# LLNL/ppo_and_friends

Hardware: AMD Instinct MI355X
Metric: env_steps_per_sec (higher is better)
Workload: dtype f32; 1 GPU; C2 CartPole-v1 MLP (4->128x3->2 actor, ->1 critic), envs_per_proc=4096, ts_per_rollout=128, fixed-length synthetic trajectories, batch_size=256, epochs_per_iter=10; parallelism=dp1, hip_graphs=True

## Files before the change

ppo_and_friends_amd/csrc/mlp_device.hpp:

```cpp
#pragma once
#include <type_traits>
#include "common.hpp"
#include <cfloat>

namespace ppoaf {

constexpr int kRows = PPOAF_UPDATE_ROWS_PER_WG;
constexpr int kMaxLayers = 8;
constexpr int kMaxOut = 16;
constexpr int kMaxAdvLds = 4096;
constexpr int kThreads = 256;

typedef float f32x4 __attribute__((ext_vector_type(4)));

struct NetDev {
    int in_dim, H, depth, out_dim, act;
    long offset, size, log_std_off;
    long offW[kMaxLayers], offB[kMaxLayers];
};

__device__ __forceinline__ float act_fwd(float z, int act) {
    if (act == PPOAF_ACT_RELU) return fmaxf(z, 0.f);
    if (act == PPOAF_ACT_LEAKY_RELU) return z > 0.f ? z : 0.01f * z;
    return tanhf(z);
// ... 63 lines not shown
#pragma unroll
    for (int c = 1; c < HT; c += 2) fr[c] = frag_u4(__builtin_amdgcn_raw_buffer_load_b128(rs, off + 64u * c, 0, 0));
}
template <int HT>
__device__ __forceinline__ void load_dgrad_frags_buf(const float* __restrict__ W, int n0, int lane, float4 (&fr)[HT]) {
    constexpr int H = 16 * HT;
    const __amdgpu_buffer_rsrc_t rs = frag_rsrc(W);
    const unsigned off = (unsigned)((4 * (lane >> 4) * H + n0 + (lane & 15)) * 4);
#pragma unroll
    for (int c = 0; c < HT; ++c) {
        const int row = 16 * c * H * 4;
        fr[c] = make_float4(__uint_as_float(__builtin_amdgcn_raw_buffer_load_b32(rs, off, row, 0)),
                            __uint_as_float(__builtin_amdgcn_raw_buffer_load_b32(rs, off, row + H * 4, 0)),
                            __uint_as_float(__builtin_amdgcn_raw_buffer_load_b32(rs, off, row + 2 * H * 4, 0)),
                            __uint_as_float(__builtin_amdgcn_raw_buffer_load_b32(rs, off, row + 3 * H * 4, 0)));
    }
}

template <int HT>
__device__ __forceinline__ f32x4 mfma_rows_x_frags(const float* __restrict__ A, int HS, int lane,
                                                   const float4 (&fr)[HT], float init) {
    const float* arow = A + (lane & 15) * HS + 4 * (lane >> 4);
    f32x4 acc0 = {init, init, init, init};
    f32x4 acc1 = {0.f, 0.f, 0.f, 0.f};
#pragma unroll
    for (int c = 0; c < HT; ++c) {
        const float4 a4 = *reinterpret_cast<const float4*>(arow + 16 * c);
        if (c & 1) {
            acc1 = __builtin_amdgcn_mfma_f32_16x16x4f32(a4.x, fr[c].x, acc1, 0, 0, 0);
            acc1 = __builtin_amdgcn_mfma_f32_16x16x4f32(a4.y, fr[c].y, acc1, 0, 0, 0);
            acc1 = __builtin_amdgcn_mfma_f32_16x16x4f32(a4.z, fr[c].z, acc1, 0, 0, 0);
            acc1 = __builtin_amdgcn_mfma_f32_16x16x4f32(a4.w, fr[c].w, acc1, 0, 0, 0);
        } else {
            acc0 = __builtin_amdgcn_mfma_f32_16x16x4f32(a4.x, fr[c].x, acc0, 0, 0, 0);
            acc0 = __builtin_amdgcn_mfma_f32_16x16x4f32(a4.y, fr[c].y, acc0, 0, 0, 0);
            acc0 = __builtin_amdgcn_mfma_f32_16x16x4f32(a4.z, fr[c].z, acc0, 0, 0, 0);
            acc0 = __builtin_amdgcn_mfma_f32_16x16x4f32(a4.w, fr[c].w, acc0, 0, 0, 0);
        }
    }
    return acc0 + acc1;
}

constexpr int kLineRow = 36;
constexpr int kLineSlot = 16 * kLineRow;
template <int HT>
__device__ __forceinline__ void load_fwd_lines_buf(const float* __restrict__ W, int n0, int lane, float4 (&raw)[HT]) {
    static_assert(HT % 2 == 0, "whole lines: H a multiple of 32");
    const __amdgpu_buffer_rsrc_t rs = frag_rsrc(W);
    const unsigned off = (unsigned)(((n0 + (lane >> 3)) * (16 * HT) + 4 * (lane & 7)) * 4);
#pragma unroll
    for (int q = 0; q < HT / 2; ++q) {
        raw[2 * q] = frag_u4(__builtin_amdgcn_raw_buffer_load_b128(rs, off + 128u * q, 0, 0));
        raw[2 * q + 1] = frag_u4(__builtin_amdgcn_raw_buffer_load_b128(rs, off + (unsigned)(8 * 16 * HT * 4) + 128u * q, 0, 0));
    }
}
template <int HT>
__device__ __forceinline__ f32x4 mfma_rows_x_lines(const float* __restrict__ A, int HS, int lane, const float4 (&raw)[HT],
                                                   float init, float* __restrict__ scratch) {
    constexpr int NL = HT / 2;
    const float* arow = A + (lane & 15) * HS + 4 * (lane >> 4);
    float* wr = scratch + (lane >> 3) * kLineRow + 4 * (lane & 7);
    const float* rd = scratch + (lane & 15) * kLineRow + 4 * (lane >> 4);
    f32x4 acc0 = {init, init, init, init};
    f32x4 acc1 = {0.f, 0.f, 0.f, 0.f};
    *reinterpret_cast<float4*>(wr) = raw[0];
    *reinterpret_cast<float4*>(wr + 8 * kLineRow) = raw[1];
    if (NL > 1) {
        *reinterpret_cast<float4*>(wr + kLineSlot) = raw[2];
        *reinterpret_cast<float4*>(wr + kLineSlot + 8 * kLineRow) = raw[3];
    }
    __builtin_amdgcn_wave_barrier();
    float4 f0 = *reinterpret_cast<const float4*>(rd);
    float4 f1 = *reinterpret_cast<const float4*>(rd + 16);
#pragma unroll
    for (int q = 0; q < NL; ++q) {
        const int slot = (q & 1) * kLineSlot;
        float4 g0 = f0, g1 = f1;
        if (q + 1 < NL) {
            g0 = *reinterpret_cast<const float4*>(rd + (kLineSlot - slot));
            g1 = *reinterpret_cast<const float4*>(rd + (kLineSlot - slot) + 16);
        }
        const float4 a0 = *reinterpret_cast<const float4*>(arow + 32 * q);
        const float4 a1 = *reinterpret_cast<const float4*>(arow + 32 * q + 16);
        acc0 = __builtin_amdgcn_mfma_f32_16x16x4f32(a0.x, f0.x, acc0, 0, 0, 0);
        acc0 = __builtin_amdgcn_mfma_f32_16x16x4f32(a0.y, f0.y, acc0, 0, 0, 0);
        acc0 = __builtin_amdgcn_mfma_f32_16x16x4f32(a0.z, f0.z, acc0, 0, 0, 0);
        acc0 = __builtin_amdgcn_mfma_f32_16x16x4f32(a0.w, f0.w, acc0, 0, 0, 0);
        acc1 = __builtin_amdgcn_mfma_f32_16x16x4f32(a1.x, f1.x, acc1, 0, 0, 0);
        acc1 = __builtin_amdgcn_mfma_f32_16x16x4f32(a1.y, f1.y, acc1, 0, 0, 0);
        acc1 = __builtin_amdgcn_mfma_f32_16x16x4f32(a1.z, f1.z, acc1, 0, 0, 0);
        acc1 = __builtin_amdgcn_mfma_f32_16x16x4f32(a1.w, f1.w, acc1, 0, 0, 0);
        __builtin_amdgcn_wave_barrier();
        if (q + 2 < NL) {
            *reinterpret_cast<float4*>(wr + slot) = raw[2 * q + 4];
            *reinterpret_cast<float4*>(wr + slot + 8 * kLineRow) = raw[2 * q + 5];
        }
        f0 = g0; f1 = g1;
    }
    return acc0 + acc1;
}

__device__ __forceinline__ void wgrad_mtile(const float* __restrict__ D, int HS, const float* __restrict__ Bsrc,
                                            int strideB, int m0, int ntiles, int n_valid, int lane,
                                            float* __restrict__ dstW, int ldw) {
    float a[4];
#pragma unroll
    for (int j = 0; j < 4; ++j) a[j] = D[(4 * (lane >> 4) + j) * HS + m0 + (lane & 15)];
    const float* bcol = Bsrc + (4 * (lane >> 4)) * strideB + (lane & 15);
    float* drow = dstW + (long)(m0 + 4 * (lane >> 4)) * ldw + (lane & 15);
#pragma unroll 4
    for (int nt = 0; nt < ntiles; ++nt) {
        f32x4 acc = {0.f, 0.f, 0.f, 0.f};
#pragma unroll
        for (int j = 0; j < 4; ++j)
            acc = __builtin_amdgcn_mfma_f32_16x16x4f32(a[j], bcol[j * strideB + 16 * nt], acc, 0, 0, 0);
        if (16 * nt + (lane & 15) < n_valid) {
#pragma unroll
            for (int r = 0; r < 4; ++r) drow[(long)r * ldw + 16 * nt] = acc[r];
        }
    }
}

template <int NT>
__device__ __forceinline__ void wgrad_mtile_full(const float* __restrict__ D, int HS, const float* __restrict__ Bsrc,
                                                 int strideB, int m0, int lane, float* __restrict__ dstW, int ldw) {
    float a[4];
#pragma unroll
    for (int j = 0; j < 4; ++j) a[j] = D[(4 * (lane >> 4) + j) * HS + m0 + (lane & 15)];
    const float* bcol = Bsrc + (4 * (lane >> 4)) * strideB + (lane & 15);
    float b[NT][4];
#pragma unroll
    for (int nt = 0; nt < NT; ++nt)
#pragma unroll
        for (int j = 0; j < 4; ++j) b[nt][j] = bcol[j * strideB + 16 * nt];
    f32x4 acc[NT];
#pragma unroll
    for (int nt = 0; nt < NT; ++nt) acc[nt] = f32x4{0.f, 0.f, 0.f, 0.f};
#pragma unroll
    for (int j = 0; j < 4; ++j)
#pragma unroll
        for (int nt = 0; nt < NT; ++nt) acc[nt] = __builtin_amdgcn_mfma_f32_16x16x4f32(a[j], b[nt][j], acc[nt], 0, 0, 0);
    float* drow = dstW + (long)(m0 + 4 * (lane >> 4)) * ldw + (lane & 15);
#pragma unroll
    for (int nt = 0; nt < NT; ++nt)
#pragma unroll
        for (int r = 0; r < 4; ++r) drow[(long)r * ldw + 16 * nt] = acc[nt][r];
}

constexpr int kNW = 8;
constexpr int kThreadsU = 64 * kNW;

template <int HT, bool ALIGNED>
__device__ __forceinline__ void load_fwd_frags_ld(const float* __restrict__ W, long ldw, int n0, int lane,
                                                  float4 (&fr)[HT]) {
    const float* w = W + (long)(n0 + (lane & 15)) * ldw + 4 * (lane >> 4);
    if (ALIGNED) {
#pragma unroll
        for (int c = 0; c < HT; c += 2) fr[c] = *reinterpret_cast<const float4*>(w + 16 * c);
        __builtin_amdgcn_sched_barrier(0);
#pragma unroll
        for (int c = 1; c < HT; c += 2) fr[c] = *reinterpret_cast<const float4*>(w + 16 * c);
    } else {
#pragma unroll
        for (int c = 0; c < HT; ++c) fr[c] = make_float4(w[16 * c], w[16 * c + 1], w[16 * c + 2], w[16 * c + 3]);
    }
}
// ... 218 lines not shown
```

ppo_and_friends_amd/csrc/ppo_update.hip:

```cpp
#include "ppo_update_fwd_bwd.hpp"
#include "peer_exchange_device.hpp"
#include <cstdlib>

namespace ppoaf {

constexpr int kRedThreads = 256;

__device__ __forceinline__ void ppo_update_bookkeeping(const UpdateDev& u);

__global__ __launch_bounds__(kRedThreads) void ppo_update_reduce_kernel(UpdateDev u, int compute_norms) {
    __shared__ double red[17];
    if (blockIdx.x == gridDim.x - 1) { ppo_update_bookkeeping(u); return; }
    const long n4 = u.bucket_total >> 2;
    const long idx = (long)blockIdx.x * kRedThreads + threadIdx.x;
    const float4* sl = reinterpret_cast<const float4*>(u.slabs);
    float4 acc = make_float4(0.f, 0.f, 0.f, 0.f);
    if (idx < n4) {
        for (int g0 = 0; g0 < u.n_wg; g0 += 8) {
            float4 v[8];
#pragma unroll
            for (int k = 0; k < 8; ++k)
                v[k] = (g0 + k < u.n_wg) ? sl[(long)(g0 + k) * n4 + idx] : make_float4(0.f, 0.f, 0.f, 0.f);
#pragma unroll
            for (int k = 0; k < 8; ++k) { acc.x += v[k].x; acc.y += v[k].y; acc.z += v[k].z; acc.w += v[k].w; }
// ... 338 lines not shown
                       dim3(kRedThreads), 0, (hipStream_t)stream, u, compute_norms);
    return check_launch("ppo_update_reduce");
}

extern "C" int ppoaf_ppo_update_reduce_exchange(const ppoaf_ppo_update_args_t* args, ppoaf_peer_exchange_t* xchg,
                                                double wait_seconds, ppoaf_stream_t stream) {
    UpdateDev u;
    int rc = make_update_dev(args, u);
    if (rc) return rc;
    PPOAF_REQUIRE(xchg && xchg->connected, "ppo_update_reduce_exchange: exchange missing or not connected");
    const long n4 = u.bucket_total >> 2;
    PPOAF_REQUIRE(xchg->dev.n4 == n4, "ppo_update_reduce_exchange: exchange made for %ld float4, bucket has %ld",
                  xchg->dev.n4, n4);
    PPOAF_REQUIRE(xchg->dev.n_ranks == u.n_ranks || !u.normalize_values, "ppo_update_reduce_exchange: %d ranks in the exchange, %d in args",
                  xchg->dev.n_ranks, u.n_ranks);
    const long groups = (n4 + kRedThreads - 1) / kRedThreads;
    PPOAF_REQUIRE(groups <= kXchgMaxGrid, "ppo_update_reduce_exchange: bucket of %ld floats needs %ld workgroups (at most %d: "
                  "use ppoaf_ppo_update_reduce + ppoaf_peer_exchange_allreduce)", (long)u.bucket_total, groups, kXchgMaxGrid);
    PPOAF_REQUIRE(wait_seconds > 0.0 && wait_seconds <= 600.0, "ppo_update_reduce_exchange: wait_seconds=%g", wait_seconds);
    hipLaunchKernelGGL(ppo_update_reduce_exchange_kernel, dim3((unsigned)groups + 1u), dim3(kRedThreads), 0,
                       (hipStream_t)stream, u, xchg->dev, (long long)(wait_seconds * 1.0e8));
    return check_launch("ppo_update_reduce_exchange");
}

extern "C" int ppoaf_ppo_update_adam(const ppoaf_ppo_update_args_t* args, int compute_norms,
                                     ppoaf_stream_t stream) {
    UpdateDev u;
    int rc = make_update_dev(args, u);
    if (rc) return rc;
    const long n4 = u.bucket_total >> 2;
    const unsigned grid = (unsigned)((n4 + 255) / 256);
    PPOAF_REQUIRE(compute_norms >= 0 && compute_norms <= 3, "ppo_update_adam: compute_norms=%d (0 .. 3)", compute_norms);
    PPOAF_REQUIRE(compute_norms != 3 || u.split, "ppo_update_adam: compute_norms = 3 follows ppoaf_ppo_update_wgrad (split_workspace set)");
    static_assert(kRedThreads == 256, "the reduce launch and the norm pass leave one partial pair per 256 float4 columns");
    if (compute_norms == 1) {
        hipLaunchKernelGGL(ppo_update_sqnorm_kernel, dim3(grid), dim3(256), 0, (hipStream_t)stream, u);
        rc = check_launch("ppo_update_adam/sqnorm");
        if (rc) return rc;
    }
    hipLaunchKernelGGL(ppo_update_adam_kernel, dim3(grid), dim3(256), 0, (hipStream_t)stream, u,
                       compute_norms == 2 ? (const double*)nullptr : (const double*)(u.norm_scratch + 6),
                       compute_norms == 3 ? (unsigned)split_wgrad_blocks(u) : grid);
    return check_launch("ppo_update_adam");
}

extern "C" int ppoaf_ppo_update_chain_allreduce(const ppoaf_ppo_update_args_t* args, ppoaf_comm_t* comm, int64_t n_minibatches,
                                                ppoaf_stream_t stream) {
    PPOAF_REQUIRE(args && comm, "ppo_update_chain_allreduce: null argument");
    PPOAF_REQUIRE(n_minibatches >= 1 && n_minibatches <= (1 << 20), "ppo_update_chain_allreduce: n_minibatches=%ld", (long)n_minibatches);
    PPOAF_REQUIRE(args->mb_offset == 0, "ppo_update_chain_allreduce: mb_offset must be 0");
    ppoaf_ppo_update_args_t a = copy_update_args(args);
    for (int64_t j = 0; j < n_minibatches; ++j) {
        a.mb_offset = j;
        a.cursor_advance = (j == n_minibatches - 1) ? n_minibatches : 0;
        int rc = ppoaf_ppo_update_fwd_bwd(&a, stream);
        if (rc == PPOAF_OK) rc = ppoaf_ppo_update_reduce(&a, 0, stream);
        if (rc == PPOAF_OK) rc = ppoaf_allreduce_sum_f32(comm, a.grads, a.bucket_total, stream);
        if (rc == PPOAF_OK) rc = ppoaf_ppo_update_adam(&a, 1, stream);
        if (rc != PPOAF_OK) return rc;
    }
    return PPOAF_OK;
}

extern "C" int ppoaf_ppo_update_adam_exchanged(const ppoaf_ppo_update_args_t* args, ppoaf_peer_exchange_t* xchg,
                                               ppoaf_stream_t stream) {
    UpdateDev u;
    int rc = make_update_dev(args, u);
    if (rc) return rc;
    PPOAF_REQUIRE(xchg && xchg->connected, "ppo_update_adam_exchanged: exchange missing or not connected");
    const long n4 = u.bucket_total >> 2;
    PPOAF_REQUIRE(xchg->dev.n4 == n4, "ppo_update_adam_exchanged: exchange made for %ld float4, bucket has %ld",
                  xchg->dev.n4, n4);
    const unsigned groups = u.split ? (unsigned)split_wgrad_blocks(u) : (unsigned)((n4 + kRedThreads - 1) / kRedThreads);
    PPOAF_REQUIRE(groups <= (unsigned)kXchgMaxGrid, "ppo_update_adam_exchanged: bucket too large for the fused exchange");
    hipLaunchKernelGGL(ppo_update_adam_kernel, dim3((unsigned)((n4 + 255) / 256)), dim3(256), 0, (hipStream_t)stream, u,
                       (const double*)xchg->dev.norm_partials, groups);
    return check_launch("ppo_update_adam_exchanged");
}

#ifdef PPOAF_STAMPS
extern "C" int ppoaf_debug_read_stamps(unsigned long long* out ) {
    return hipMemcpyFromSymbol(out, HIP_SYMBOL(g_ppo_update_stamps), sizeof(unsigned long long) * 32) == hipSuccess ? 0 : -2;
}
#endif

extern "C" int ppoaf_minibatch_moments(const float* data, const int64_t* perm, const int32_t* row_map,
                                       int64_t n_perm, int64_t B, double* records,
                                       ppoaf_stream_t stream) {
    PPOAF_REQUIRE(data && perm && records, "minibatch_moments: null pointer");
    PPOAF_REQUIRE(n_perm >= 1 && B >= 1, "minibatch_moments: n_perm=%ld B=%ld", (long)n_perm, (long)B);
    const long nb = (n_perm + B - 1) / B;
    PPOAF_REQUIRE(nb <= 0x7fffffffL, "minibatch_moments: too many mini-batches");
    hipLaunchKernelGGL(minibatch_moments_kernel, dim3((unsigned)nb), dim3(256), 0, (hipStream_t)stream,
                       data, perm, row_map, (long)n_perm, (long)B, records);
    return check_launch("minibatch_moments");
}
```

ppo_and_friends_amd/csrc/ppo_update_dev.hpp:

```cpp
#pragma once
#include "action_heads.hpp"
#include "running_stats_device.hpp"
#include "wgrad_tile.hpp"
#include <cstddef>
#include <cstring>

namespace ppoaf {

#ifdef PPOAF_STAMPS
#ifndef PPOAF_STAMP_BLOCK
#define PPOAF_STAMP_BLOCK 0
#endif
static __device__ unsigned long long g_ppo_update_stamps[2][16];
#define PPOAF_STAMP_AT(row, k, t0)                                                       \
    do {                                                                                 \
        if (blockIdx.x == PPOAF_STAMP_BLOCK && threadIdx.x == (t0)) {                    \
            unsigned long long t_;                                                       \
            asm volatile("s_memtime %0\n\ts_waitcnt lgkmcnt(0)" : "=s"(t_)::"memory");    \
            g_ppo_update_stamps[row][k] = t_;                                            \
        }                                                                                \
    } while (0)
#define PPOAF_STAMP(k) PPOAF_STAMP_AT(0, k, 0)
#define PPOAF_STAMP_W(k, w) PPOAF_STAMP_AT(1, k, 64 * (w))
#else
#define PPOAF_STAMP(k) do {} while (0)
#define PPOAF_STAMP_W(k, w) do {} while (0)
#endif

#define PPOAF_WIDTH_PAIRS_IN_UPDATE(X) X(32, 32) X(64, 64) X(128, 128) X(256, 256) X(128, 256) X(64, 128)
#define PPOAF_WIDTH_PAIRS_IN_NARROW(X) X(64, 256) X(32, 256) X(32, 64)
#define PPOAF_WIDTH_PAIRS_WIDE(X) X(256, 512)
#define PPOAF_WIDTH_PAIRS_EVERY_FORM(X) PPOAF_WIDTH_PAIRS_IN_UPDATE(X) PPOAF_WIDTH_PAIRS_IN_NARROW(X)
#define PPOAF_WIDTH_PAIRS(X) PPOAF_WIDTH_PAIRS_EVERY_FORM(X) PPOAF_WIDTH_PAIRS_WIDE(X)
#define PPOAF_WIDTH_PAIR_RUNG_(A, C) if (ppoaf_ha_ == A && ppoaf_hc_ == C) return PPOAF_WIDTH_PAIR_CALL_(A, C);
#define PPOAF_WIDTH_PAIR_LADDER_OF(LIST, ha, hc) \
    { const int ppoaf_ha_ = (ha), ppoaf_hc_ = (hc); LIST(PPOAF_WIDTH_PAIR_RUNG_) }
#define PPOAF_WIDTH_PAIR_LADDER(ha, hc) PPOAF_WIDTH_PAIR_LADDER_OF(PPOAF_WIDTH_PAIRS_EVERY_FORM, ha, hc)
#define PPOAF_WIDTH_PAIR_LADDER_ALL(ha, hc) PPOAF_WIDTH_PAIR_LADDER_OF(PPOAF_WIDTH_PAIRS, ha, hc)
inline bool width_pair_instantiated(const int ha, const int hc) {
#define PPOAF_WIDTH_PAIR_CALL_(A, C) true
    PPOAF_WIDTH_PAIR_LADDER_ALL(ha, hc)
#undef PPOAF_WIDTH_PAIR_CALL_
    return false;
}
inline bool width_pair_is_wide(const int ha, const int hc) {
#define PPOAF_WIDTH_PAIR_CALL_(A, C) true
    PPOAF_WIDTH_PAIR_LADDER_OF(PPOAF_WIDTH_PAIRS_WIDE, ha, hc)
#undef PPOAF_WIDTH_PAIR_CALL_
    return false;
}
inline size_t rowtile_wide_lds_floats(const NetDev& n) {
    const size_t HS = n.H + 4, INP = 16 * ((n.in_dim + 15) / 16) + 4;
    return 208 + (size_t)(n.depth + 1) * n.H + (size_t)n.H + kRows * INP + 3 * kRows * HS + 2 * kRows * kMaxOut;
}

struct WsDev {
    float* hbuf[2];
    float* dbuf[2];
    float* outpart[2];
    float* xbuf[2];
    int W;
    int xld[2];
    int Bp;
};

struct UpdateDev {
    NetDev net[2];
    const float* params; float* grads; float* exp_avg; float* exp_avg_sq; float* slabs;
    long bucket_total;
    int64_t* step_counts; const float* lr; double* norm_scratch;
    float beta1, beta2, adam_eps, grad_scale, max_norm; int head_kind;
    const float* obs; const float* critic_obs; const void* raw_actions;
    const float* adv; const float* old_lp; const float* rtg; float* values;
    const int64_t* perm; const int32_t* row_map; long n_rows;
    int64_t* cursor; long B, batch_stride, mb_offset, cursor_advance;
    int normalize_values, n_ranks;
    float* vn_mean; float* vn_var; double* vn_count; const double* vn_records;
    const double* adv_records;
    int normalize_adv, use_huber, pregathered;
    float surr_clip, entropy_weight, kl_loss_weight, huber_delta, min_std;
    float* loss_partials; double* totals;
    int n_wg;
    int confine;
    int split;
    WsDev sp;
    int n_slices; int slices[8];
};

inline long ws_seg_off(const NetDev& n) {
    const long szW0 = ((long)n.H * n.in_dim + 3) & ~3L;
    return n.depth == 0 ? 0 : szW0 + n.H + (long)(n.depth - 1) * ((long)n.H * n.H + n.H);
}
inline long ws_seg_len(const NetDev& n) { return n.size - ws_seg_off(n); }

inline int split_wgrad_jobs(const NetDev& n) {
    const int t = n.H / 16, t2 = (t + 1) / 2, p0 = ((n.in_dim + 15) / 16 + 1) / 2;
    return (n.depth - 1) * t * t2 + t * p0 + 1;
}
inline int split_wgrad_per_xcd(const UpdateDev& u) { return (split_wgrad_jobs(u.net[0]) + split_wgrad_jobs(u.net[1]) + 7) / 8; }
inline int split_wgrad_blocks(const UpdateDev& u) { return 8 * split_wgrad_per_xcd(u); }

inline bool args_row_pairs(const ppoaf_ppo_update_args_t* a) { return (a->row_pairs & PPOAF_SPLIT_ROW_PAIRS) != 0; }
inline bool args_wide_inputs(const ppoaf_ppo_update_args_t* a) { return (a->row_pairs & PPOAF_SPLIT_WIDE_INPUTS) != 0; }

inline int split_xld(const NetDev& n) { return n.in_dim <= 64 ? 64 : 128; }

inline size_t ws_layout(const UpdateDev& u, WsDev* ws, char* base) {
    const long Bp = (u.B + 63) & ~63L;
    size_t off = 0;
// ... 382 lines not shown
```

ppo_and_friends_amd/csrc/ppo_update_rowtile.hpp:

```cpp
#pragma once
#include "ppo_update_dev.hpp"

namespace ppoaf {

extern __shared__ __attribute__((aligned(16))) unsigned char ppo_update_smem[];




__device__ __forceinline__ int rowtile_request_args(const UpdateDev& u, int b) {
    const NetDev& a = u.net[0];
    const NetDev& c = u.net[1];
    asm("" : "+s"(b)
        : "s"(a.in_dim), "s"(a.H), "s"(a.depth), "s"(a.out_dim), "s"(a.act), "s"((&a.act)[1]), "s"(a.offset), "s"(a.size), "s"(a.log_std_off),
          "s"(c.in_dim), "s"(c.H), "s"(c.depth), "s"(c.out_dim), "s"(c.act), "s"((&c.act)[1]), "s"(c.offset), "s"(c.size), "s"(c.log_std_off),
          "s"(u.params), "s"(u.norm_scratch), "s"(u.head_kind),
          "s"(u.obs), "s"(u.critic_obs), "s"(u.raw_actions), "s"(u.adv), "s"(u.old_lp), "s"(u.rtg), "s"(u.values), "s"(u.perm),
          "s"(u.row_map), "s"(u.n_rows), "s"(u.cursor), "s"(u.B), "s"(u.batch_stride), "s"(u.mb_offset), "s"(u.cursor_advance),
          "s"(u.normalize_values), "s"(u.n_ranks), "s"(u.vn_mean), "s"(u.vn_var), "s"(u.vn_count), "s"(u.vn_records),
          "s"(u.adv_records), "s"(u.normalize_adv), "s"(u.use_huber), "s"(u.pregathered), "s"(u.surr_clip),
          "s"(u.n_wg), "s"(u.confine));
    const long cur = u.cursor[0];
    asm("" : "+s"(b)
        : "s"(cur), "s"(u.entropy_weight), "s"(u.kl_loss_weight), "s"(u.huber_delta), "s"(u.min_std), "s"(u.loss_partials),
          "s"(u.sp.hbuf[0]), "s"(u.sp.hbuf[1]), "s"(u.sp.dbuf[0]), "s"(u.sp.dbuf[1]), "s"(u.sp.outpart[0]), "s"(u.sp.outpart[1]),
          "s"(u.sp.xbuf[0]), "s"(u.sp.xbuf[1]), "s"(u.sp.W), "s"(u.sp.xld[0]), "s"(u.sp.xld[1]), "s"(u.sp.Bp), "s"(u.n_slices),
          "s"(u.slices[0]), "s"(u.slices[1]), "s"(u.slices[2]), "s"(u.slices[3]), "s"(u.slices[4]), "s"(u.slices[5]),
          "s"(u.slices[6]), "s"(u.slices[7]));
    return b;
}

template <int CP> __device__ __forceinline__ void lds_read_adjacent(const float* p, float (&v)[CP]) {
    if constexpr (CP % 4 == 0) {
#pragma unroll
        for (int q = 0; q < CP / 4; ++q) {
            const float4 t = *reinterpret_cast<const float4*>(p + 4 * q);
            v[4 * q] = t.x; v[4 * q + 1] = t.y; v[4 * q + 2] = t.z; v[4 * q + 3] = t.w;
        }
    } else {
#pragma unroll
        for (int q = 0; q < CP; ++q) v[q] = p[q];
    }
}
template <int CP> __device__ __forceinline__ void lds_write_adjacent(float* p, const float (&v)[CP]) {
    if constexpr (CP % 4 == 0) {
#pragma unroll
        for (int q = 0; q < CP / 4; ++q) *reinterpret_cast<float4*>(p + 4 * q) = make_float4(v[4 * q], v[4 * q + 1], v[4 * q + 2], v[4 * q + 3]);
    } else {
#pragma unroll
        for (int q = 0; q < CP; ++q) p[q] = v[q];
    }
}

template <int HT, bool SPLIT, bool TABLES, bool XLD = false>
__device__ __forceinline__ void ppo_update_fwd_bwd_body_as(const UpdateDev& u, const int which, const int g) {
    constexpr int H = 16 * HT, HS = H + 4;
    const int tid = threadIdx.x, lane = tid & 63, wave = tid >> 6;
    const auto& nd = u.net[which];
    const int in_dim = nd.in_dim, depth = nd.depth, out_dim = nd.out_dim, act = nd.act;
    const int NT0 = (in_dim + 15) >> 4;
    const int INP = 16 * NT0 + 4;
    const float* P = u.params + nd.offset;
    const long B = u.B;
    const long mb = u.cursor[0] + u.mb_offset;
    const long base = mb * u.batch_stride;
    const long szW0 = ((long)H * in_dim + 3) & ~3L;
    auto offW = [&](int l) -> long { return l == 0 ? 0 : szW0 + H + (long)(l - 1) * (H * H + H); };
    auto offB = [&](int l) -> long {
        return l == 0 ? szW0 : offW(l) + (l < depth ? (long)H * H : (((long)out_dim * H + 3) & ~3L));
    };
    float* slab = SPLIT ? u.sp.outpart[which] + (long)g * (nd.size - offW(depth)) - offW(depth)
                        : u.slabs + (long)g * u.bucket_total + nd.offset;
    constexpr int kPub = (kRows * (H / 4) + kThreadsU - 1) / kThreadsU;
    constexpr bool kPubLate = HT <= kNW;
    float4 pub[kPub];
    auto publish_read = [&](const float* src) {
#pragma unroll
        for (int q = 0; q < kPub; ++q) {
            const int i = tid + q * kThreadsU, r = i / (H / 4), c4 = i - r * (H / 4);
            if (i < kRows * (H / 4)) pub[q] = *reinterpret_cast<const float4*>(src + r * HS + 4 * c4);
        }
    };
    auto publish_store = [&](float* panel) {
        float* dst = panel + (long)g * kRows * H;
#pragma unroll
        for (int q = 0; q < kPub; ++q) {
            const int i = tid + q * kThreadsU, r = i / (H / 4), c4 = i - r * (H / 4);
            if (i < kRows * (H / 4)) *reinterpret_cast<float4*>(dst + (long)r * H + 4 * c4) = pub[q];
        }
    };
    auto publish_begin = [&](const float* src, float* panel) {
        publish_read(src);
        if constexpr (!kPubLate) publish_store(panel);
    };
    auto publish_end = [&](float* panel) {
        if constexpr (kPubLate) { __builtin_amdgcn_sched_barrier(0); publish_store(panel); }
    };
    const long sp_plane = SPLIT ? (long)u.sp.Bp * H : 0;

    PPOAF_STAMP(0);
    float* smem = reinterpret_cast<float*>(ppo_update_smem);
    int* sRow = reinterpret_cast<int*>(smem);
    float* sMisc = smem + 16;
    float* sRowF = smem + 32;
    float* sActF = smem + 80;
    float* sBias = smem + 208;
    float* sWout = sBias + (depth + 1) * H;
    float* sX = sWout + 8 * H;
    float* sH = sX + kRows * INP;
    float* sD0 = sH + (long)depth * kRows * HS;
    float* sD1 = sD0 + kRows * HS;
    float* sOut = sD1 + kRows * HS;
    float* sDOut = sOut + kRows * kMaxOut;
    float* sScr = sDOut + kRows * kMaxOut + wave * 2 * kLineSlot;

    if (g == 0 && which == 0 && tid == 0) { u.norm_scratch[0] = 0.0; u.norm_scratch[1] = 0.0; }

    const bool has_tile = HT >= kNW || wave < HT;
    static_assert(!TABLES || HT <= kNW, "deep prefetch: one output tile per wave");
    const bool deep = TABLES || (depth == 3 && HT <= kNW);
    float4 fr[HT], fr2[HT];
    const bool l0_pre = in_dim <= 16 && HT <= kNW && has_tile;
    float l0w[4] = {0.f, 0.f, 0.f, 0.f};
    float l2_touch = 0.f;
    constexpr int kCopyRegs = 4;
    float bias_reg[kCopyRegs], wout_reg[kCopyRegs];
    const int n_bias = (depth + 1) * H, n_wout = out_dim * H;
    const bool copy_fits = n_bias <= kCopyRegs * kThreadsU && n_wout <= kCopyRegs * kThreadsU;
    auto request_weights = [&]() {
        (void)fr; (void)fr2;
        if (l0_pre) {
            const float* w = P + offW(0) + (long)(wave * 16 + (lane & 15)) * in_dim;
#pragma unroll
            for (int j = 0; j < 4; ++j) { const int k = 4 * j + (lane >> 4); if (k < in_dim) l0w[j] = w[k]; }
        }
#ifndef PPOAF_L2_TOUCH_MAX_HT
#define PPOAF_L2_TOUCH_MAX_HT 8
#endif
        if (!deep && HT <= PPOAF_L2_TOUCH_MAX_HT) for (long i = (long)tid * 32; i < nd.size; i += (long)kThreadsU * 32) l2_touch += P[i];
        if (copy_fits) {
#pragma unroll
            for (int r = 0; r < kCopyRegs; ++r) {
                const int i = tid + r * kThreadsU;
                bias_reg[r] = 0.f; wout_reg[r] = 0.f;
                if (i < n_bias) { const int l = i / H, j = i - l * H; if (l < depth || j < out_dim) bias_reg[r] = P[offB(l) + j]; }
                if (i < n_wout) wout_reg[r] = P[offW(depth) + i];
            }
        }
    };
    auto request_hidden_sets = [&]() {
        if (deep && has_tile) {
            load_fwd_lines_buf<HT>(P + offW(1), wave * 16, lane, fr);
            load_fwd_lines_buf<HT>(P + offW(2), wave * 16, lane, fr2);
        }
    };
    const float* x_src = which == 0 ? u.obs : u.critic_obs;
    const bool x_pre = (TABLES || u.pregathered) && kRows * in_dim <= 2 * kThreadsU;
    float xr[2] = {0.f, 0.f};
    if (x_pre) {
#pragma unroll
        for (int q = 0; q < 2; ++q) {
            const int idx = tid + q * kThreadsU;
            if (idx < kRows * in_dim && (long)g * kRows + idx / in_dim < B) xr[q] = x_src[(base + (long)g * kRows) * in_dim + idx];
        }
    }
    if constexpr (TABLES) asm volatile("; ppoaf_rowtile_tables_prologue");
    request_weights();

    constexpr int kActRegs = 8;
    constexpr int kVnPre = 2;
    const bool row_lane = tid < kRows && (long)g * kRows + tid < B;
    constexpr bool early = TABLES;
    const int n_act = which != 0 ? 0 : u.head_kind == PPOAF_HEAD_CATEGORICAL ? 1
                    : u.head_kind == PPOAF_HEAD_MULTI_CATEGORICAL ? u.n_slices : out_dim;
    long perm_v = -1;
    float av = 0.f, lpo = 0.f, rt = 0.f;
    int act_bits[kActRegs];
#pragma unroll
    for (int j = 0; j < kActRegs; ++j) act_bits[j] = 0;
    auto request_row_scalars = [&](const long di) {
        if (which == 0) {
            av = u.adv[di]; lpo = u.old_lp[di];
            if (u.head_kind == PPOAF_HEAD_CATEGORICAL) {
// ... 114 lines not shown
                    m = new_mean; v = (float)(m_2 / (cnt + n)); cnt = new_count;
                }
            }
            sMisc[2] = m; sMisc[3] = v;
            if (g == 0) { u.vn_mean[slot ^ 1] = m; u.vn_var[slot ^ 1] = v; u.vn_count[slot ^ 1] = cnt; }
        }
    }
    if (copy_fits) {
#pragma unroll
        for (int r = 0; r < kCopyRegs; ++r) {
            const int i = tid + r * kThreadsU;
            if (i < n_bias) sBias[i] = bias_reg[r];
            if (i < n_wout) sWout[i] = wout_reg[r];
        }
    } else {
        for (int l = 0; l <= depth; ++l) {
            const int n = (l == depth) ? out_dim : H;
            const float* bb = P + offB(l);
            for (int i = tid; i < n; i += kThreadsU) sBias[l * H + i] = bb[i];
        }
        for (int i = tid; i < out_dim * H; i += kThreadsU) sWout[i] = P[offW(depth) + i];
    }
    for (int i = tid; i < kRows * INP; i += kThreadsU) sX[i] = 0.f;
    __syncthreads();
    PPOAF_STAMP(1);

    if (x_pre) {
#pragma unroll
        for (int q = 0; q < 2; ++q) {
            const int idx = tid + q * kThreadsU;
            const int s = idx / in_dim, i = idx - s * in_dim;
            if (idx < kRows * in_dim && sRow[s] >= 0) sX[s * INP + i] = xr[q];
        }
    } else {
        const float* src = x_src;
        for (int idx = tid; idx < kRows * in_dim; idx += kThreadsU) {
            const int s = idx / in_dim, i = idx - s * in_dim;
            const int row = sRow[s];
            const long di = (TABLES || u.pregathered) ? base + (long)g * kRows + s : row;
            if (row >= 0) sX[s * INP + i] = src[di * in_dim + i];
        }
    }
    if (!deep && depth > 1 && has_tile) load_fwd_lines_buf<HT>(P + offW(1), wave * 16, lane, fr);
    __syncthreads();
    PPOAF_STAMP(2);
    if constexpr (SPLIT && XLD) {
        const int xld = u.sp.xld[which], sh = xld == 64 ? 6 : 7;
        float* xb = u.sp.xbuf[which] + (long)g * kRows * xld;
        for (int i = tid; i < kRows * xld; i += kThreadsU) {
            const int r = i >> sh, c = i & (xld - 1);
            xb[i] = c < 16 * NT0 ? sX[r * INP + c] : 0.f;
        }
    } else if (SPLIT) {
        float* xb = u.sp.xbuf[which] + (long)g * kRows * 64;
        for (int i = tid; i < kRows * 64; i += kThreadsU) {
            const int r = i >> 6, c = i & 63;
            xb[i] = c < 16 * NT0 ? sX[r * INP + c] : 0.f;
        }
    }

    for (int nt = wave; nt < HT; nt += kNW) {
        const int o = nt * 16 + (lane & 15);
        const float bv = sBias[o];
        f32x4 acc = {bv, bv, bv, bv};
        const float* w = P + offW(0) + (long)o * in_dim;
        const float* arow = sX + (lane & 15) * INP;
        for (int k0 = 0; k0 < in_dim; k0 += 16) {
            float bq[4];
#pragma unroll
            for (int j = 0; j < 4; ++j) {
                const int k = k0 + 4 * j + (lane >> 4);
                bq[j] = l0_pre ? l0w[j] : (k < in_dim ? w[k] : 0.f);
            }
#pragma unroll
            for (int j = 0; j < 4; ++j)
                acc = __builtin_amdgcn_mfma_f32_16x16x4f32(arow[k0 + 4 * j + (lane >> 4)], bq[j], acc, 0, 0, 0);
        }
#pragma unroll
        for (int r = 0; r < 4; ++r) sH[(4 * (lane >> 4) + r) * HS + o] = act_fwd(acc[r], act);
    }
    __syncthreads();
    PPOAF_STAMP(3);

    for (int l = 1; l < depth; ++l) {
        const float* Hp = sH + (long)(l - 1) * kRows * HS;
        float* Hc = sH + (long)l * kRows * HS;
        if (SPLIT) publish_begin(Hp, u.sp.hbuf[which] + (long)(l - 1) * sp_plane);
        for (int nt = wave; nt < HT; nt += kNW) {
            const int o = nt * 16 + (lane & 15);
            f32x4 acc;
            if (deep) {
                if (l == 1) {
                    acc = mfma_rows_x_lines<HT>(Hp, HS, lane, fr, sBias[l * H + o], sScr);
                    load_dgrad_frags<HT>(P + offW(2), wave * 16, lane, fr);
                } else {
                    acc = mfma_rows_x_lines<HT>(Hp, HS, lane, fr2, sBias[l * H + o], sScr);
                    load_dgrad_frags<HT>(P + offW(1), wave * 16, lane, fr2);
                }
            } else {
            if (nt != wave) load_fwd_lines_buf<HT>(P + offW(l), nt * 16, lane, fr);
            acc = mfma_rows_x_lines<HT>(Hp, HS, lane, fr, sBias[l * H + o], sScr);
            if (nt + kNW >= HT) {
                if (l + 1 < depth) load_fwd_lines_buf<HT>(P + offW(l + 1), wave * 16, lane, fr);
                else load_dgrad_frags<HT>(P + offW(l), wave * 16, lane, fr);
            }
            }
#pragma unroll
            for (int r = 0; r < 4; ++r) Hc[(4 * (lane >> 4) + r) * HS + o] = act_fwd(acc[r], act);
        }
        if (SPLIT) publish_end(u.sp.hbuf[which] + (long)(l - 1) * sp_plane);
        __syncthreads();
    }
    PPOAF_STAMP(4);
    const float* Hlast = sH + (long)(depth - 1) * kRows * HS;

    if (tid < 256) {
        const int s = tid >> 4, part = tid & 15;
        for (int k = 0; k < out_dim; ++k) {
            float acc = 0.f;
#pragma unroll
            for (int i = 0; i < HT; ++i) acc = fmaf(Hlast[s * HS + part + 16 * i], sWout[k * H + part + 16 * i], acc);
            acc = group16_sum(acc);
            if (part == 0) sOut[s * kMaxOut + k] = acc + sBias[depth * H + k];
        }
    }
    __syncthreads();
    PPOAF_STAMP(5);

    if (wave == 0) {
        if constexpr (TABLES) asm volatile("; ppoaf_rowtile_head_rows_begin");
        ppo_head_rows(u, which, out_dim, P + nd.log_std_off, sRow, sRowF, sMisc, sActF, sOut, sDOut, lane, B);
        if constexpr (TABLES) asm volatile("; ppoaf_rowtile_head_rows_end");
        PPOAF_STAMP_W(0, 0);
    }
    __syncthreads();
    if constexpr (TABLES) asm volatile("; ppoaf_rowtile_middle_begin");
    PPOAF_STAMP(6);

    {
        constexpr int CP = H / 32;
        static_assert(kThreadsU == 32 * kRows && H % 32 == 0, "dz_last: 32 lane groups per row");
        const int s = tid >> 5, c0 = (tid & 31) * CP;
        float d[8];
        const float4 d0 = *reinterpret_cast<const float4*>(sDOut + s * kMaxOut);
        const float4 d1 = *reinterpret_cast<const float4*>(sDOut + s * kMaxOut + 4);
        d[0] = d0.x; d[1] = d0.y; d[2] = d0.z; d[3] = d0.w; d[4] = d1.x; d[5] = d1.y; d[6] = d1.z; d[7] = d1.w;
        float hv[CP], acc[CP], wv[CP];
        lds_read_adjacent<CP>(Hlast + s * HS + c0, hv);
#pragma unroll
        for (int ii = 0; ii < CP; ++ii) acc[ii] = 0.f;
#pragma unroll
        for (int k = 0; k < 8; ++k) {
            if (k < out_dim) {
                lds_read_adjacent<CP>(sWout + k * H + c0, wv);
#pragma unroll
                for (int ii = 0; ii < CP; ++ii) acc[ii] = fmaf(d[k], wv[ii], acc[ii]);
            }
        }
#pragma unroll
        for (int ii = 0; ii < CP; ++ii) acc[ii] = acc[ii] * act_bwd(hv[ii], act);
        lds_write_adjacent<CP>(sD0 + s * HS + c0, acc);
    }
    PPOAF_STAMP_W(2, 0); PPOAF_STAMP_W(3, 4); PPOAF_STAMP_W(4, 5);
    if constexpr (TABLES) asm volatile("; ppoaf_rowtile_middle_end");
    __syncthreads();
    PPOAF_STAMP(7);

    float* Dc = sD0;
    float* Dn = sD1;
    for (int l = depth - 1; l >= 1; --l) {
        const float* Hin = sH + (long)(l - 1) * kRows * HS;
        if (SPLIT) publish_begin(Dc, u.sp.dbuf[which] + (long)l * sp_plane);
        for (int nt = wave; nt < HT; nt += kNW) {
            f32x4 acc;
            if (deep) {
                acc = l == 2 ? mfma_rows_x_frags<HT>(Dc, HS, lane, fr, 0.f) : mfma_rows_x_frags<HT>(Dc, HS, lane, fr2, 0.f);
            } else {
            if (nt != wave) load_dgrad_frags<HT>(P + offW(l), nt * 16, lane, fr);
            acc = mfma_rows_x_frags<HT>(Dc, HS, lane, fr, 0.f);
            if (nt + kNW >= HT && l - 1 >= 1) load_dgrad_frags<HT>(P + offW(l - 1), wave * 16, lane, fr);
            }
#pragma unroll
            for (int r = 0; r < 4; ++r) {
                const int s = 4 * (lane >> 4) + r, i = nt * 16 + (lane & 15);
                Dn[s * HS + i] = acc[r] * act_bwd(Hin[s * HS + i], act);
            }
        }
        if (SPLIT) publish_end(u.sp.dbuf[which] + (long)l * sp_plane);
        if (l == depth - 1) PPOAF_STAMP(10);
        if (!SPLIT) {
            for (int mt = wave; mt < HT; mt += kNW) {
                if (HT <= 8) wgrad_mtile_full<(HT <= 8 ? HT : 1)>(Dc, HS, Hin, HS, mt * 16, lane, slab + offW(l), H);
                else wgrad_mtile(Dc, HS, Hin, HS, mt * 16, HT, H, lane, slab + offW(l), H);
            }
            if (l == depth - 1) PPOAF_STAMP(11);
            for (int o = tid; o < H; o += kThreadsU) {
                float acc = 0.f;
#pragma unroll
                for (int s = 0; s < kRows; ++s) acc += Dc[s * HS + o];
                slab[offB(l) + o] = acc;
            }
        }
        if (l == depth - 1) PPOAF_STAMP(12);
        __syncthreads();
        if (l == depth - 1) PPOAF_STAMP(13);
        float* t = Dc; Dc = Dn; Dn = t;
    }
    PPOAF_STAMP(8);

    if (SPLIT) {
        publish_read(Dc);
        publish_store(u.sp.dbuf[which]);
    } else {
        for (int mt = wave; mt < HT; mt += kNW)
            wgrad_mtile(Dc, HS, sX, INP, mt * 16, NT0, in_dim, lane, slab + offW(0), in_dim);
        for (int o = tid; o < H; o += kThreadsU) {
            float acc = 0.f;
#pragma unroll
            for (int s = 0; s < kRows; ++s) acc += Dc[s * HS + o];
            slab[offB(0) + o] = acc;
        }
    }
    PPOAF_STAMP_W(6, 0);

    if (tid < H) {
        const int i = tid;
        float h[kRows];
#pragma unroll
        for (int s = 0; s < kRows; ++s) h[s] = Hlast[s * HS + i];
        for (int k = 0; k < out_dim; ++k) {
            float d[kRows];
#pragma unroll
            for (int s = 0; s < kRows; ++s) d[s] = sDOut[s * kMaxOut + k];
            float acc = 0.f;
#pragma unroll
            for (int s = 0; s < kRows; ++s) acc = fmaf(d[s], h[s], acc);
            slab[offW(depth) + (long)k * H + i] = acc;
        }
    }
    {
        const int out_pad = SPLIT ? ((out_dim + 3) & ~3) : out_dim;
        if (tid >= 256 && tid < 256 + out_pad) {
            const int k = tid - 256;
            float acc = 0.f;
            if (k < out_dim) {
#pragma unroll
                for (int s = 0; s < kRows; ++s) acc += sDOut[s * kMaxOut + k];
            }
            slab[offB(depth) + k] = acc;
// ... 38 lines not shown
```

Baseline: 1.161 million env-steps/s.

## Pace next-layer weight loads inside hidden forward MFMA loop and defer dgrad fragment loads

Result: faster. 1.199 million env-steps/s (median of 6 runs) (+3.3%).

```diff
diff --git a/ppo_and_friends_amd/csrc/mlp_device.hpp b/ppo_and_friends_amd/csrc/mlp_device.hpp
--- a/ppo_and_friends_amd/csrc/mlp_device.hpp
+++ b/ppo_and_friends_amd/csrc/mlp_device.hpp
@@ -169,6 +169,60 @@
         }
         const float4 a0 = *reinterpret_cast<const float4*>(arow + 32 * q);
         const float4 a1 = *reinterpret_cast<const float4*>(arow + 32 * q + 16);
+        acc0 = __builtin_amdgcn_mfma_f32_16x16x4f32(a0.x, f0.x, acc0, 0, 0, 0);
+        acc0 = __builtin_amdgcn_mfma_f32_16x16x4f32(a0.y, f0.y, acc0, 0, 0, 0);
+        acc0 = __builtin_amdgcn_mfma_f32_16x16x4f32(a0.z, f0.z, acc0, 0, 0, 0);
+        acc0 = __builtin_amdgcn_mfma_f32_16x16x4f32(a0.w, f0.w, acc0, 0, 0, 0);
+        acc1 = __builtin_amdgcn_mfma_f32_16x16x4f32(a1.x, f1.x, acc1, 0, 0, 0);
+        acc1 = __builtin_amdgcn_mfma_f32_16x16x4f32(a1.y, f1.y, acc1, 0, 0, 0);
+        acc1 = __builtin_amdgcn_mfma_f32_16x16x4f32(a1.z, f1.z, acc1, 0, 0, 0);
+        acc1 = __builtin_amdgcn_mfma_f32_16x16x4f32(a1.w, f1.w, acc1, 0, 0, 0);
+        __builtin_amdgcn_wave_barrier();
+        if (q + 2 < NL) {
+            *reinterpret_cast<float4*>(wr + slot) = raw[2 * q + 4];
+            *reinterpret_cast<float4*>(wr + slot + 8 * kLineRow) = raw[2 * q + 5];
+        }
+        f0 = g0; f1 = g1;
+    }
+    return acc0 + acc1;
+}
+template <int HT>
+__device__ __forceinline__ f32x4 mfma_rows_x_lines_paced(const float* __restrict__ A, int HS, int lane, float4 (&raw)[HT],
+                                                         float init, float* __restrict__ scratch, const float* __restrict__ Wd,
+                                                         int n0) {
+    constexpr int NL = HT / 2, H = 16 * HT;
+    const float* arow = A + (lane & 15) * HS + 4 * (lane >> 4);
+    float* wr = scratch + (lane >> 3) * kLineRow + 4 * (lane & 7);
+    const float* rd = scratch + (lane & 15) * kLineRow + 4 * (lane >> 4);
+    const float* wd = Wd + (long)(4 * (lane >> 4)) * H + n0 + (lane & 15);
+    f32x4 acc0 = {init, init, init, init};
+    f32x4 acc1 = {0.f, 0.f, 0.f, 0.f};
+    *reinterpret_cast<float4*>(wr) = raw[0];
+    *reinterpret_cast<float4*>(wr + 8 * kLineRow) = raw[1];
+    if (NL > 1) {
+        *reinterpret_cast<float4*>(wr + kLineSlot) = raw[2];
+        *reinterpret_cast<float4*>(wr + kLineSlot + 8 * kLineRow) = raw[3];
+    }
+    __builtin_amdgcn_wave_barrier();
+    float4 f0 = *reinterpret_cast<const float4*>(rd);
+    float4 f1 = *reinterpret_cast<const float4*>(rd + 16);
+#pragma unroll
+    for (int q = 0; q < NL; ++q) {
+        const int slot = (q & 1) * kLineSlot;
+        float4 g0 = f0, g1 = f1;
+        if (q + 1 < NL) {
+            g0 = *reinterpret_cast<const float4*>(rd + (kLineSlot - slot));
+            g1 = *reinterpret_cast<const float4*>(rd + (kLineSlot - slot) + 16);
+        }
+        const float4 a0 = *reinterpret_cast<const float4*>(arow + 32 * q);
+        const float4 a1 = *reinterpret_cast<const float4*>(arow + 32 * q + 16);
+        __builtin_amdgcn_sched_barrier(0);
+#pragma unroll
+        for (int p = 0; p < 2; ++p) {
+            const float* wp = wd + (long)(16 * (2 * q + p)) * H;
+            raw[2 * q + p] = make_float4(wp[0], wp[H], wp[2 * H], wp[3 * H]);
+        }
+        __builtin_amdgcn_sched_barrier(0);
         acc0 = __builtin_amdgcn_mfma_f32_16x16x4f32(a0.x, f0.x, acc0, 0, 0, 0);
         acc0 = __builtin_amdgcn_mfma_f32_16x16x4f32(a0.y, f0.y, acc0, 0, 0, 0);
         acc0 = __builtin_amdgcn_mfma_f32_16x16x4f32(a0.z, f0.z, acc0, 0, 0, 0);
diff --git a/ppo_and_friends_amd/csrc/ppo_update.hip b/ppo_and_friends_amd/csrc/ppo_update.hip
--- a/ppo_and_friends_amd/csrc/ppo_update.hip
+++ b/ppo_and_friends_amd/csrc/ppo_update.hip
@@ -444,6 +444,9 @@
 extern "C" int ppoaf_debug_read_stamps(unsigned long long* out ) {
     return hipMemcpyFromSymbol(out, HIP_SYMBOL(g_ppo_update_stamps), sizeof(unsigned long long) * 32) == hipSuccess ? 0 : -2;
 }
+extern "C" int ppoaf_debug_read_hidden_stamps(unsigned long long* out ) {
+    return hipMemcpyFromSymbol(out, HIP_SYMBOL(g_ppo_hidden_stamps), sizeof(unsigned long long) * 128) == hipSuccess ? 0 : -2;
+}
 #endif
 
 extern "C" int ppoaf_minibatch_moments(const float* data, const int64_t* perm, const int32_t* row_map,
diff --git a/ppo_and_friends_amd/csrc/ppo_update_dev.hpp b/ppo_and_friends_amd/csrc/ppo_update_dev.hpp
--- a/ppo_and_friends_amd/csrc/ppo_update_dev.hpp
+++ b/ppo_and_friends_amd/csrc/ppo_update_dev.hpp
@@ -22,9 +22,26 @@
     } while (0)
 #define PPOAF_STAMP(k) PPOAF_STAMP_AT(0, k, 0)
 #define PPOAF_STAMP_W(k, w) PPOAF_STAMP_AT(1, k, 64 * (w))
+static __device__ unsigned long long g_ppo_hidden_stamps[2][8][8];
+#define PPOAF_HSTAMP_DECL unsigned long long hstamp_[8] = {0, 0, 0, 0, 0, 0, 0, 0}
+#define PPOAF_HSTAMP(k)                                                                  \
+    do {                                                                                 \
+        __builtin_amdgcn_sched_barrier(0);                                               \
+        asm volatile("s_memtime %0\n\ts_waitcnt lgkmcnt(0)" : "=s"(hstamp_[k])::"memory"); \
+        __builtin_amdgcn_sched_barrier(0);                                               \
+    } while (0)
+#define PPOAF_HSTAMP_FLUSH(layer)                                                        \
+    do {                                                                                 \
+        if (blockIdx.x == PPOAF_STAMP_BLOCK && (threadIdx.x & 63) == 0) {                \
+            for (int k_ = 0; k_ < 8; ++k_) g_ppo_hidden_stamps[layer][threadIdx.x >> 6][k_] = hstamp_[k_]; \
+        }                                                                                \
+    } while (0)
 #else
 #define PPOAF_STAMP(k) do {} while (0)
 #define PPOAF_STAMP_W(k, w) do {} while (0)
+#define PPOAF_HSTAMP_DECL do {} while (0)
+#define PPOAF_HSTAMP(k) do {} while (0)
+#define PPOAF_HSTAMP_FLUSH(layer) do {} while (0)
 #endif
 
 #define PPOAF_WIDTH_PAIRS_IN_UPDATE(X) X(32, 32) X(64, 64) X(128, 128) X(256, 256) X(128, 256) X(64, 128)
diff --git a/ppo_and_friends_amd/csrc/ppo_update_rowtile.hpp b/ppo_and_friends_amd/csrc/ppo_update_rowtile.hpp
--- a/ppo_and_friends_amd/csrc/ppo_update_rowtile.hpp
+++ b/ppo_and_friends_amd/csrc/ppo_update_rowtile.hpp
@@ -99,6 +99,7 @@
     const long sp_plane = SPLIT ? (long)u.sp.Bp * H : 0;
 
     PPOAF_STAMP(0);
+    PPOAF_HSTAMP_DECL;
     float* smem = reinterpret_cast<float*>(ppo_update_smem);
     int* sRow = reinterpret_cast<int*>(smem);
     float* sMisc = smem + 16;
@@ -379,10 +380,33 @@
     __syncthreads();
     PPOAF_STAMP(3);
 
+    if constexpr (TABLES) asm volatile("; ppoaf_rowtile_hidden_fwd_begin" ::: "memory");
     for (int l = 1; l < depth; ++l) {
+        if constexpr (TABLES) asm volatile("; ppoaf_rowtile_hidden_layer_begin" ::: "memory");
         const float* Hp = sH + (long)(l - 1) * kRows * HS;
         float* Hc = sH + (long)l * kRows * HS;
         if (SPLIT) publish_begin(Hp, u.sp.hbuf[which] + (long)(l - 1) * sp_plane);
+        PPOAF_HSTAMP(0);
+        if constexpr (TABLES) {
+            if (has_tile) {
+                const int o = wave * 16 + (lane & 15);
+                const float bv = sBias[l * H + o];
+                f32x4 acc;
+                if (wave == 0) {
+                    if (l == 1) acc = mfma_rows_x_lines_paced<HT>(Hp, HS, lane, fr, bv, sScr, P + offW(2), wave * 16);
+                    else acc = mfma_rows_x_lines_paced<HT>(Hp, HS, lane, fr2, bv, sScr, P + offW(1), wave * 16);
+                } else {
+                    acc = l == 1 ? mfma_rows_x_lines<HT>(Hp, HS, lane, fr, bv, sScr) : mfma_rows_x_lines<HT>(Hp, HS, lane, fr2, bv, sScr);
+                }
+                PPOAF_HSTAMP(1);
+#pragma unroll
+                for (int r = 0; r < 4; ++r) Hc[(4 * (lane >> 4) + r) * HS + o] = act_fwd(acc[r], act);
+                asm volatile("; ppoaf_rowtile_hidden_epilogue_end" ::: "memory");
+            }
+            if (SPLIT) publish_end(u.sp.hbuf[which] + (long)(l - 1) * sp_plane);
+            PPOAF_HSTAMP(3);
+            PPOAF_HSTAMP(2);
+        } else {
         for (int nt = wave; nt < HT; nt += kNW) {
             const int o = nt * 16 + (lane & 15);
             f32x4 acc;
@@ -406,11 +430,20 @@
             for (int r = 0; r < 4; ++r) Hc[(4 * (lane >> 4) + r) * HS + o] = act_fwd(acc[r], act);
         }
         if (SPLIT) publish_end(u.sp.hbuf[which] + (long)(l - 1) * sp_plane);
+        }
         __syncthreads();
+        PPOAF_HSTAMP(4);
+        PPOAF_HSTAMP_FLUSH(l - 1);
     }
     PPOAF_STAMP(4);
     const float* Hlast = sH + (long)(depth - 1) * kRows * HS;
 
+    if constexpr (TABLES) {
+        if (has_tile && wave >= 4) {
+            load_dgrad_frags<HT>(P + offW(2), wave * 16, lane, fr);
+            load_dgrad_frags<HT>(P + offW(1), wave * 16, lane, fr2);
+        }
+    }
     if (tid < 256) {
         const int s = tid >> 4, part = tid & 15;
         for (int k = 0; k < out_dim; ++k) {
@@ -429,6 +462,12 @@
         ppo_head_rows(u, which, out_dim, P + nd.log_std_off, sRow, sRowF, sMisc, sActF, sOut, sDOut, lane, B);
         if constexpr (TABLES) asm volatile("; ppoaf_rowtile_head_rows_end");
         PPOAF_STAMP_W(0, 0);
+    }
+    if constexpr (TABLES) {
+        if (has_tile && wave >= 1 && wave < 4) {
+            load_dgrad_frags<HT>(P + offW(2), wave * 16, lane, fr);
+            load_dgrad_frags<HT>(P + offW(1), wave * 16, lane, fr2);
+        }
     }
     __syncthreads();
     if constexpr (TABLES) asm volatile("; ppoaf_rowtile_middle_begin");
@@ -462,6 +501,7 @@
     if constexpr (TABLES) asm volatile("; ppoaf_rowtile_middle_end");
     __syncthreads();
     PPOAF_STAMP(7);
+    if constexpr (TABLES) asm volatile("; ppoaf_rowtile_hidden_bwd_begin" ::: "memory");
 
     float* Dc = sD0;
     float* Dn = sD1;
```
